# norlab-ulaval/norlab_icp_mapper

Measured on AMD Instinct MI355X. Metric: ICP iterations/sec, 100k-pt scan vs 1M-pt map, higher is better.
Workload: dtype f32; 1 GPU; single synthetic 100000-pt scan vs 1000000-pt map, point-to-point ICP, KDTreeMatcher knn 1 maxDist 2.0 epsilon 0, TrimmedDist 0.85, fixed 20 iterations per registration; chain=p2p, scene=box+pillars sigma=0.01 seeds 42/43/44 (SURVEY.md 8d), parallelism=scan-sharded x1, map replicated

## Files before the change

norlab_icp_mapper_amd/csrc/api.hip:

```cpp
#include "common.h"
#include <cstring>
#include <new>
#include <dlfcn.h>
#include <mutex>
#include <cstdio>

static std::string g_create_error;

namespace {
struct Roctx {
    int (*push)(const char*) = nullptr;
    int (*pop)() = nullptr;
    Roctx()
    {
        const char* e = getenv("ICPMI_ROCTX");
        if (!e || !atoi(e)) return;
        for (const char* name : {"librocprofiler-sdk-roctx.so.1", "librocprofiler-sdk-roctx.so", "/opt/rocm/lib/librocprofiler-sdk-roctx.so.1",
                                 "libroctx64.so.4", "libroctx64.so", "/opt/rocm/lib/libroctx64.so.4"}) {
            void* lib = dlopen(name, RTLD_NOW | RTLD_GLOBAL);
            if (!lib) continue;
            push = (int (*)(const char*))dlsym(lib, "roctxRangePushA");
            pop = (int (*)())dlsym(lib, "roctxRangePop");
            if (push && pop) return;
            push = nullptr; pop = nullptr;
// ... 213 lines not shown
icpmi_status icpmi_trim_cache(void)
{
    dev_cache_trim();
    return ICPMI_OK;
}


const char* icpmi_last_error(icpmi_handle h) { return h ? h->last_error.c_str() : g_create_error.c_str(); }

icpmi_status icpmi_set_stream(icpmi_handle h, void* hip_stream)
{
    CHECK_H(h);
    if (h->stream) hipStreamSynchronize(h->stream);
    if (h->own_stream && h->stream) stream_release(h->stream);
    h->stream = (hipStream_t)hip_stream;
    h->own_stream = false;
    drop_loop_graphs(h);
    return ICPMI_OK;
}

int32_t icpmi_has_map(icpmi_handle h) { return h && h->m > 0 ? 1 : 0; }

icpmi_status icpmi_get_map_mean(icpmi_handle h, float mean3[3])
{
    if (!h || !mean3) return ICPMI_ERR_INVALID_ARG;
    memcpy(mean3, h->mean, 3 * sizeof(float));
    return ICPMI_OK;
}

icpmi_status icpmi_debug_counters(icpmi_handle h, uint64_t out[24])
{
    if (!h || !out) return ICPMI_ERR_INVALID_ARG;
    for (int i = 0; i < 24; ++i) out[i] = h->h_state->dbg[i];
#ifndef ICPMI_NN_TIMING
    out[14] = (uint64_t)h->merge_fast_epochs;
    out[15] = (uint64_t)h->merge_slow_epochs;
    out[16] = (uint64_t)h->oct_respeculated;
    out[17] = (uint64_t)h->raw_view_count;
    out[18] = (uint64_t)(uint32_t)h->ins_count | ((uint64_t)(uint32_t)(h->temp_raw ? h->temp_raw->ins_count : 0) << 32);
    out[19] = (uint64_t)(uint32_t)h->full_count | ((uint64_t)(uint32_t)(h->temp_raw ? h->temp_raw->full_count : 0) << 32);
    out[20] = (uint64_t)h->normals_incremental;
    out[21] = (uint64_t)h->normals_full;
    out[22] = (uint64_t)h->normals_last_searched;
#endif
    return ICPMI_OK;
}

icpmi_status icpmi_debug_last_matches(icpmi_handle h, int64_t n, int32_t k, int32_t* ids, float* d2, float T_used[16])
{
    CHECK_H(h);
    if (n < 1 || k < 1 || !ids || !d2 || !T_used) { h->last_error = "debug_last_matches: bad arguments"; return ICPMI_ERR_INVALID_ARG; }
    if (h->last_match_n == 0) {
        h->last_error = "debug_last_matches: no single registration's matches on this handle (none ran, it failed, or a batch / another call came after it)";
        return ICPMI_ERR_UNSUPPORTED;
    }
    if (n != h->last_match_n || k != h->last_match_k) { h->last_error = "debug_last_matches: n / k differ from the last registration's"; return ICPMI_ERR_INVALID_ARG; }
    const size_t cnt = (size_t)n * k;
    DevBuf<int> d_ids;
    HIP_TRY(h, d_ids.alloc(cnt));
    icpmi_status s = nn_ids_to_original(h, h->d_sidx, (int64_t)cnt, d_ids);
    if (s != ICPMI_OK) return s;
    std::vector<int> hid(cnt), hq(h->last_match_sorted ? (size_t)n : 0);
    std::vector<float> hd(cnt);
    HIP_TRY(h, hipMemcpyAsync(hid.data(), d_ids, cnt * sizeof(int), hipMemcpyDeviceToHost, h->stream));
    HIP_TRY(h, hipMemcpyAsync(hd.data(), h->d_d2, cnt * sizeof(float), hipMemcpyDeviceToHost, h->stream));
    if (h->last_match_sorted) HIP_TRY(h, hipMemcpyAsync(hq.data(), h->d_qindex, (size_t)n * sizeof(int), hipMemcpyDeviceToHost, h->stream));
    HIP_TRY(h, hipMemcpyAsync(T_used, h->d_state->T_prev, 16 * sizeof(float), hipMemcpyDeviceToHost, h->stream));
// ... 766 lines not shown
```

norlab_icp_mapper_amd/csrc/common.h:

```cpp
#pragma once

#include <hip/hip_runtime.h>
#include <stdint.h>
#include <math.h>
#include <cstring>
#include <string>
#include <vector>
#include <unordered_map>
#include <mutex>
#include <map>
#include <cstdlib>
#include <shared_mutex>

#include "../../include/icpmi.h"

#define ICPMI_NV 32
#define ICPMI_MAX_OUTLIER 8
#define ICPMI_MAX_SMOOTH 16
#define ICPMI_SEL_BINS 2048
#ifndef ICPMI_S2_COPIES
#define ICPMI_S2_COPIES 8
#endif
#define ICPMI_S2_C0 4096
#define ICPMI_S2_F0 (ICPMI_S2_C0 + ICPMI_S2_COPIES * 256)
// ... 121 lines not shown
    int   stop_reason;
    int   counter;
    int   hist_n;
    double hq[(ICPMI_MAX_SMOOTH + 1) * 4];
    double ht[(ICPMI_MAX_SMOOTH + 1) * 3];
    double hrot[ICPMI_MAX_SMOOTH + 1];
    double htr[ICPMI_MAX_SMOOTH + 1];
    double init_q[4];
    unsigned sel_prefix;
    unsigned sel_rank;
    unsigned n_valid;
    unsigned sel_prefix_l[3];
    unsigned sel_rank_l[3];
    float limits[ICPMI_MAX_OUTLIER];
    unsigned vt_valid;
    float vt_ratio;
    float robust_med;
    float robust_scale;
    long long pairs;
    double wsum;
    unsigned hard_count;
    unsigned ticket;
    unsigned long long hard_total;
    unsigned seq;
    unsigned long long dbg[24];
    float T_prev[16];
    float T_out[16];
    unsigned long long t_start, t_done;
    unsigned long long t_nn_begin, t_nn_sum;
    unsigned nn_count, pad_nn;
};

#ifdef __HIPCC__
__device__ __forceinline__ void nn_stamp_open(IcpState* st) { st->t_nn_begin = (unsigned long long)wall_clock64(); }
__device__ __forceinline__ void nn_stamp_close(IcpState* st)
{
    const unsigned long long b = st->t_nn_begin;
    if (b) { st->t_nn_sum += (unsigned long long)wall_clock64() - b; ++st->nn_count; st->t_nn_begin = 0; }
}
#endif


inline std::shared_mutex& capture_gate() { static std::shared_mutex* m = new std::shared_mutex; return *m; }
struct CaptureGate {
    CaptureGate() { capture_gate().lock_shared(); }
    ~CaptureGate() { capture_gate().unlock_shared(); }
    CaptureGate(const CaptureGate&) = delete;
    CaptureGate& operator=(const CaptureGate&) = delete;
};

struct LoopGraph {
    hipGraphExec_t exec = nullptr; uint64_t sig = 0; int uses = 0; bool sorted = false;
    int len = 0; unsigned long used = 0;
    bool holds(uint64_t s) const { return exec && sig == s; }
    void reset() { if (exec) hipGraphExecDestroy(exec); *this = LoopGraph(); }
};
struct LoopGraphs {
    LoopGraph fixed, batch, seg[2], heads[4];
    unsigned long clock = 0;
    void reset() { fixed.reset(); batch.reset(); for (LoopGraph& g : seg) g.reset(); for (LoopGraph& g : heads) g.reset(); }
};

struct DevBlockCache {
    struct Live { size_t bytes; int dev; };
    std::mutex mu;
    std::unordered_map<void*, Live> live;
    std::map<int, std::multimap<size_t, void*>> idle_of;
// ... 616 lines not shown
```

norlab_icp_mapper_amd/csrc/loop.hip:

```cpp
#include "common.h"
#include "solve.h"
#include <cstring>

namespace {

template <int PASS, int MODE = 0>
__global__ __launch_bounds__(256) void sel_hist_kernel(const float* __restrict__ d2, int64_t count,
                                                       const IcpState* __restrict__ st, unsigned* __restrict__ ghist, int nb_scale = 0)
{
    if (st->done) return;
    if (blockIdx.x == 0 && threadIdx.x == 0) nn_stamp_close(const_cast<IcpState*>(st));
    if (MODE != 0 && nb_scale != 0 && st->iter + 1 > nb_scale) return;
    if (MODE == 3 && st->iter != 0) return;
    __shared__ unsigned h[ICPMI_SEL_BINS];
    for (int b = threadIdx.x; b < ICPMI_SEL_BINS; b += 256) h[b] = 0;
    __syncthreads();
    const unsigned prefix = st->sel_prefix;
    const float med = MODE == 2 ? st->robust_med : 0.f;
    for (int64_t i = (int64_t)blockIdx.x * 256 + threadIdx.x; i < count; i += (int64_t)gridDim.x * 256) {
        float v = d2[i];
        if (MODE == 0 || MODE == 3) { if (!(v != INFINITY && v > 0.f)) continue; }
        else {
            if (v == INFINITY) continue;
            if (MODE == 2) v = fabsf(v - med);
// ... 268 lines not shown
    for (int u = 0; u < PF; ++u) add(pv[u]);
    for (int64_t i = i0 + PF * stride; i < count; i += stride) add(d2[i]);
    __syncthreads();
    for (int i = threadIdx.x; i < WIN; i += 256) {
        const unsigned cnt = win[i];
        if (cnt) { const unsigned bin = lo + (unsigned)i; atomicAdd(&h[bin >> 8], cnt); atomicAdd(&fine[ICPMI_S2_FIDX(bin)], cnt); }
    }
    __syncthreads();
    if (h[threadIdx.x]) atomicAdd(&hists[ICPMI_S2_C0 + (blockIdx.x % ICPMI_S2_COPIES) * 256 + threadIdx.x], h[threadIdx.x]);
}

__global__ __launch_bounds__(256) void sel2_scan_hist_kernel(const float* __restrict__ d2, BatchArgs ba, int k, IcpState* __restrict__ st,
                                                             unsigned* __restrict__ hists, float quantile, int use_win)
{
    const int64_t count = (int64_t)ba.n[blockIdx.y] * k;
    d2 += (size_t)blockIdx.y * (size_t)ba.qstride * k;
    hists += (size_t)blockIdx.y * ICPMI_SELHIST_WORDS;
    st += blockIdx.y;
    constexpr int PF = 2;
    const int64_t stride = (int64_t)gridDim.x * 256;
    const int64_t i0 = (int64_t)blockIdx.x * 256 + threadIdx.x;
    float pv[PF];
#pragma unroll
    for (int u = 0; u < PF; ++u) pv[u] = i0 + u * stride < count ? d2[i0 + u * stride] : INFINITY;
    unsigned cv = 0;
#pragma unroll
    for (int cpy = 0; cpy < ICPMI_S2_COPIES; ++cpy) cv += hists[ICPMI_S2_C0 + cpy * 256 + threadIdx.x];
    if (st->done) return;
    if (blockIdx.x == 0 && threadIdx.x == 0) nn_stamp_close(const_cast<IcpState*>(st));
    __shared__ unsigned sh[16];
    unsigned prefix, rem, total;
    const bool win_hit = use_win && win_lookup(hists, quantile, sh, prefix, rem, total);
    if (!win_hit) block_find_rank_2tier<ICPMI_S2_FCOPIES>(cv, hists + ICPMI_S2_F0, true, quantile, 0u, sh, prefix, rem, total);
#ifndef ICPMI_NN_TIMING
    if (use_win && blockIdx.x == 0 && threadIdx.x == 0) st->dbg[win_hit ? 12 : 13] += 1ull;
#endif
    if (total == 0) {
        if (blockIdx.x == 0 && threadIdx.x == 0) { st->n_valid = 0; st->error = ICPMI_ERR_NO_OUTLIER_TO_FILTER; st->done = 1; }
        return;
    }
    if (blockIdx.x == 0 && threadIdx.x == 0) { st->sel_prefix_l[0] = prefix; st->sel_rank_l[0] = rem; st->n_valid = total; }
    auto add = [&](float v) {
        if (!(v != INFINITY && v > 0.f)) return;
        const unsigned bits = __float_as_uint(v);
        if ((bits >> 16) != prefix) return;
        atomicAdd(&hists[ICPMI_S2_C1 + ((bits >> 8) & 255u)], 1u);
        atomicAdd(&hists[ICPMI_S2_F1 + ICPMI_S2_FIDX(bits & 0xffffu)], 1u);
    };
#pragma unroll
    for (int u = 0; u < PF; ++u) add(pv[u]);
    for (int64_t i = i0 + PF * stride; i < count; i += stride) add(d2[i]);
}

constexpr int VT_CHUNK = 2048;

__global__ __launch_bounds__(256) void vt_keys_kernel(const float* __restrict__ d2, int64_t count, IcpState* __restrict__ st,
                                                      unsigned long long* __restrict__ keys, unsigned* __restrict__ vals)
{
    const int64_t i = (int64_t)blockIdx.x * 256 + threadIdx.x;
    if (blockIdx.x == 0 && threadIdx.x == 0 && !st->done) nn_stamp_close(st);
    const float v = i < count ? d2[i] : INFINITY;
    const bool valid = v != INFINITY && v > 0.f;
    if (i < count) { keys[i] = valid ? (unsigned long long)__float_as_uint(v) : 0xffffffffull; vals[i] = 0u; }
    __shared__ unsigned cnt;
    if (threadIdx.x == 0) cnt = 0;
    __syncthreads();
    const unsigned long long b = __ballot(valid);
// ... 1537 lines not shown
```

norlab_icp_mapper_amd/csrc/nn.hip:

```cpp
#include "common.h"

namespace {

constexpr int NN_BLOCK = 256;

typedef __attribute__((address_space(1))) unsigned gunsigned;
__device__ __forceinline__ float sqrt_up(float x) { return __builtin_amdgcn_sqrtf(x) * 1.0000005f; }
typedef float vf4 __attribute__((ext_vector_type(4)));
typedef __attribute__((address_space(1))) vf4 gfloat4;

struct Cand {
    unsigned long long key;
    int sidx;
};

__device__ __forceinline__ void cand_min(Cand& a, unsigned long long key, int sidx)
{
    if (key < a.key) { a.key = key; a.sidx = sidx; }
}

template <int G>
__device__ __forceinline__ void group_reduce(Cand& c)
{
#pragma unroll
// ... 249 lines not shown
__global__ __launch_bounds__(256) void ids_kernel(const float4* __restrict__ map, const int* __restrict__ sidx, int64_t count,
                                                  int* __restrict__ ids)
{
    const int64_t i = (int64_t)blockIdx.x * 256 + threadIdx.x;
    if (i >= count) return;
    const int s = sidx[i];
    ids[i] = s < 0 ? -1 : (int)__float_as_uint(map[s].w);
}

#ifdef ICPMI_NN_TIMING
#define NN_TICK(i) do { __builtin_amdgcn_s_waitcnt(0); const long long t_ = clock64(); tacc[i] += t_ - tlast; tlast = t_; } while (0)
#else
#define NN_TICK(i) do { } while (0)
#endif
__device__ __forceinline__ unsigned wave_incl_scan(unsigned v)
{
    v += (unsigned)__builtin_amdgcn_update_dpp(0, (int)v, 0x111, 0xf, 0xf, false);
    v += (unsigned)__builtin_amdgcn_update_dpp(0, (int)v, 0x112, 0xf, 0xf, false);
    v += (unsigned)__builtin_amdgcn_update_dpp(0, (int)v, 0x114, 0xf, 0xf, false);
    v += (unsigned)__builtin_amdgcn_update_dpp(0, (int)v, 0x118, 0xf, 0xf, false);
    v += (unsigned)__builtin_amdgcn_update_dpp(0, (int)v, 0x142, 0xa, 0xf, false);
    v += (unsigned)__builtin_amdgcn_update_dpp(0, (int)v, 0x143, 0xc, 0xf, false);
    return v;
}

#ifndef ICPMI_NN1_WAVES
#define ICPMI_NN1_WAVES 7
#endif
#if ICPMI_NN1_WAVES > 0
#define NN1_WAVES_ATTR __attribute__((amdgpu_waves_per_eu(ICPMI_NN1_WAVES, ICPMI_NN1_WAVES)))
#else
#define NN1_WAVES_ATTR
#endif
template <int NW, bool SELF>
__global__ __launch_bounds__(64 * NW) NN1_WAVES_ATTR void nn1_wg_kernel(const float4* __restrict__ queries, const int* __restrict__ qindex, BatchArgs ba,
                                                     const float* __restrict__ Tptr, GridLevels L, float maxr2, int* __restrict__ out_sidx,
                                                     float* __restrict__ out_d2, IcpState* __restrict__ st, unsigned* __restrict__ hard,
                                                     unsigned* __restrict__ hist0, float4* __restrict__ match_pt,
                                                     const uint4* __restrict__ ltab_g, int unseeded_lev, int seed_pre, float inv1e, float err2)
{
    static_assert(NW == 3 || NW == 4, "waves per workgroup");
    constexpr int NT = 64 * NW, Q = 64;
    constexpr int NR = 3;
    constexpr int CAP = 16 * Q;
#ifndef ICPMI_NN1_PLB
#define ICPMI_NN1_PLB 4
#endif
    constexpr int PLB = ICPMI_NN1_PLB;
    const int n = ba.n[blockIdx.y];
    {
        const size_t qo = (size_t)blockIdx.y * (size_t)ba.qstride;
        queries += qo; out_sidx += qo; out_d2 += qo;
        if (qindex) qindex += qo;
        if (match_pt) match_pt += qo;
        if (hist0) hist0 += (size_t)blockIdx.y * ICPMI_SELHIST_WORDS;
        if (Tptr) Tptr = reinterpret_cast<const float*>(reinterpret_cast<const char*>(Tptr) + (size_t)blockIdx.y * sizeof(IcpState));
        st += blockIdx.y;
    }
#ifdef ICPMI_NN_TIMING
    long long tacc[8] = {0, 0, 0, 0, 0, 0, 0, 0};
    long long tlast = clock64();
    const long long t_c0 = tlast, t_w0 = wall_clock64();
#endif
    __shared__ uint4 ltab[ICPMI_MAXLEV * 4];
    __shared__ unsigned lh[256];
    __shared__ uint2 pieces[CAP];
    __shared__ float2 qdec[Q];
    __shared__ float4 qrec[Q];
    __shared__ float2 qaux[Q];
    __shared__ unsigned long long qkey[Q];
    __shared__ unsigned qwin[Q];
    __shared__ float4 qpt[Q];
    __shared__ unsigned s_any, s_total[2];
    const int tid = threadIdx.x;
    const int lane = tid & 63;
    const int wave = tid >> 6;
    const bool w0 = wave == 0;
#ifndef ICPMI_NN_NO_HOIST
    {
        const GridParams g0 = L.g[0];
        asm volatile("" ::"s"(queries), "s"(qindex), "s"(out_sidx), "s"(out_d2), "s"(match_pt), "s"(ltab_g), "s"(Tptr), "s"(st), "s"(hist0), "s"(hard));
        asm volatile("" ::"s"(g0.ox), "s"(g0.oy), "s"(g0.oz), "s"(g0.cell), "s"(g0.inv_cell), "s"(g0.slack), "s"(L.nlev), "s"(maxr2), "s"(unseeded_lev), "s"(seed_pre), "s"(inv1e), "s"(err2));
    }
#endif
    const int wgs = (int)((((long long)n + Q - 1) / Q + 7) / 8 * 8);
    if ((int)blockIdx.x >= wgs) return;
    const int chunk = wgs >> 3;
    const int lb = (blockIdx.x & 7) * chunk + (blockIdx.x >> 3);
    const int slot = lane;
    const int qi = lb * Q + slot;
    const bool active = w0 && qi < n;
    float4 r = make_float4(0.f, 0.f, 0.f, 1.f);
    int orig = 0, sp_kept = -1;
    float4 qs_kept = make_float4(0.f, 0.f, 0.f, 0.f);
    if (w0) {
        r = ld_stream(queries + (active ? qi : 0));
        orig = match_pt ? qi : (qindex ? qindex[active ? qi : 0] : qi);
        if (match_pt) { sp_kept = ld_stream(out_sidx + (active ? qi : 0)); qs_kept = ld_stream(match_pt + (active ? qi : 0)); }
    }
    const int st_done = st->done, st_iter = st->iter;
    uint4 ltab_mine = make_uint4(0u, 0u, 0u, 0u);
    if (tid < ICPMI_MAXLEV * 4) ltab_mine = ltab_g[tid];
    float3 p = make_float3(0.f, 0.f, 0.f);
    if (w0) {
        if (Tptr) p = xf_point(Tptr, r.x, r.y, r.z, r.w);
        else p = make_float3(r.x, r.y, r.z);
    }
    if (st_done) return;
    if (blockIdx.x == 0 && threadIdx.x == 0) nn_stamp_open(st);
    if (tid < ICPMI_MAXLEV * 4) ltab[tid] = ltab_mine;
    if (hist0) {
        for (int t = tid; t < 256; t += NT) lh[t] = 0;
        for (int gt = blockIdx.x * NT + tid; gt < 256 + 65536; gt += wgs * NT) hist0[ICPMI_S2_C1 + gt] = 0;
    }
    const bool allow_self = SELF;

    Cand best; best.key = ~0ull; best.sidx = -1;
    bool decided = !active;
    int lev0 = unseeded_lev;
    if (w0) {
        int sp = -1;
        float4 qs = make_float4(0.f, 0.f, 0.f, 0.f);
        if (active && allow_self && st_iter > 0) {
            sp = match_pt ? sp_kept : out_sidx[orig];
            if (sp >= 0) qs = match_pt ? qs_kept : L.pts[0][sp];
        }
        bool want = sp >= 0;
        const float ub2 = sqdist3(p.x, p.y, p.z, qs.x, qs.y, qs.z);
        const float ub = sqrt_up(ub2);
        auto try_level = [&](int lev, const GridParams& gl) {
            const float fx = (p.x - gl.ox) * gl.inv_cell, fy = (p.y - gl.oy) * gl.inv_cell, fz = (p.z - gl.oz) * gl.inv_cell;
            float mfl = fminf(fx - floorf(fx), 1.0f - (fx - floorf(fx)));
            mfl = fminf(mfl, fminf(fy - floorf(fy), 1.0f - (fy - floorf(fy))));
            mfl = fminf(mfl, fminf(fz - floorf(fz), 1.0f - (fz - floorf(fz))));
            if (!(mfl >= 0.f)) mfl = 0.f;
            const float margin = (1.0f + mfl) * gl.cell - 2.0f * gl.slack;
            if (want && ub * inv1e * 1.000001f <= margin) {
                lev0 = lev;
                best.key = pack_key(ub2, __float_as_uint(qs.w));
                best.sidx = sp;
                qpt[slot] = qs;
                want = false;
            }
        };
        try_level(0, L.g[0]);
        for (int lev = 1; lev < L.nlev; ++lev) {
            if (__ballot(want) == 0ull) break;
            try_level(lev, L.g[lev]);
        }
    }
    bool widepre = false;
    if (seed_pre && lev0 > 0 && best.key != ~0ull) { widepre = true; lev0 = 0; }

    int lev = lev0;
    bool did_pre = false;
    if (w0) { qrec[slot] = make_float4(p.x, p.y, p.z, __int_as_float(lev0)); qkey[slot] = best.key; qwin[slot] = (unsigned)best.sidx; }
    NN_TICK(0);
    __syncthreads();
    for (;;) {
        bool run = false, prescan = false;
        if (w0) {
            run = !decided && lev < L.nlev;
            const bool any = __ballot(run) != 0ull;
            if (lane == 0) { s_any = any ? 1u : 0u; s_total[0] = 0u; s_total[1] = 0u; }
            if (any) {
                const int lv = run ? lev : 0;
                const unsigned long long bk = qkey[slot];
                prescan = run && !did_pre && (bk == ~0ull || (widepre && lev == 0));
                float rub2 = INFINITY;
                if (!prescan && bk != ~0ull) {
                    const float slack = __uint_as_float(ltab[4 * lv + 1].y);
                    const float rub = sqrt_up(__uint_as_float((unsigned)(bk >> 32))) * inv1e * 1.000001f + slack;
                    rub2 = rub * rub;
                }
                reinterpret_cast<float*>(&qrec[slot])[3] = __int_as_float(lv);
                qaux[slot] = make_float2(rub2, __int_as_float((run ? 1 : 0) | (prescan ? 2 : 0)));
            }
        }
        __syncthreads();
        if (!s_any) break;
        NN_TICK(1);
        {
            float mf, g_cell, g_slack;
            bool covers;
            const float4 qr = qrec[slot];
            const float2 qa = qaux[slot];
            const int lv = __float_as_int(qr.w);
            const int fl = __float_as_int(qa.y);
            const bool qrun = (fl & 1) != 0, qpre = (fl & 2) != 0;
            const float rub2 = qa.x;
            GridParams g;
            const gunsigned* __restrict__ cs;
            {
                const uint4 a = ltab[4 * lv], b = ltab[4 * lv + 1], c2 = ltab[4 * lv + 2], d = ltab[4 * lv + 3];
                g.ox = __uint_as_float(a.x); g.oy = __uint_as_float(a.y); g.oz = __uint_as_float(a.z); g.cell = __uint_as_float(a.w);
                g.inv_cell = __uint_as_float(b.x); g.slack = __uint_as_float(b.y); g.nx = (int)b.z; g.ny = (int)b.w;
                g.nz = (int)c2.x; g.ncells = (int)c2.y;
                cs = reinterpret_cast<const gunsigned*>(((unsigned long long)d.y << 32) | d.x);
            }
            const float fx = (qr.x - g.ox) * g.inv_cell, fy = (qr.y - g.oy) * g.inv_cell, fz = (qr.z - g.oz) * g.inv_cell;
            const float flx = floorf(fx), fly = floorf(fy), flz = floorf(fz);
            const int cx = (int)fminf(fmaxf(flx, -1.0e6f), 1.0e6f);
            const int cy = (int)fminf(fmaxf(fly, -1.0e6f), 1.0e6f);
            const int cz = (int)fminf(fmaxf(flz, -1.0e6f), 1.0e6f);
            mf = fminf(fx - flx, 1.0f - (fx - flx));
            mf = fminf(mf, fminf(fy - fly, 1.0f - (fy - fly)));
            mf = fminf(mf, fminf(fz - flz, 1.0f - (fz - flz)));
            if (!(mf >= 0.f)) mf = 0.f;
            g_cell = g.cell; g_slack = g.slack;
            covers = cx - 1 <= 0 && cx + 1 >= g.nx - 1 && cy - 1 <= 0 && cy + 1 >= g.ny - 1 && cz - 1 <= 0 && cz + 1 >= g.nz - 1;
            if (w0) { const float margin = fmaxf((1.0f + mf) * g_cell - g_slack, 0.f); qdec[slot] = make_float2(margin * margin, covers ? 1.f : 0.f); }
            unsigned rs[NR], rn[NR];
            {
                const float ylo = (fy - fly) * g.cell, yhi = (1.0f - (fy - fly)) * g.cell;
                const float zlo = (fz - flz) * g.cell, zhi = (1.0f - (fz - flz)) * g.cell;
                unsigned ia[NR], ib[NR];
#pragma unroll
                for (int sl = 0; sl < NR; ++sl) {
                    const int rr = wave + sl * NW;
                    const int dy = (rr % 3) - 1, dz = (rr / 3) - 1;
                    bool reach = qrun && rr < 9 && (!qpre || rr == 4);
                    const float ddy = dy == 0 ? 0.f : (dy < 0 ? ylo : yhi);
                    const float ddz = dz == 0 ? 0.f : (dz < 0 ? zlo : zhi);
                    const float rem2 = rub2 - (ddy * ddy + ddz * ddz);
                    reach = reach && rem2 >= 0.f;
                    int xa = cx - 1, xb = cx + 1;
                    if (rem2 != INFINITY) {
                        const float rem = sqrt_up(fmaxf(rem2, 0.f));
                        const int xl = (int)fmaxf(floorf((qr.x - rem - g.ox) * g.inv_cell), -1.0e6f);
                        const int xh = (int)fminf(floorf((qr.x + rem - g.ox) * g.inv_cell), 1.0e6f);
                        xa = xl > xa ? xl : xa;
                        xb = xh < xb ? xh : xb;
                    }
                    const int y = cy + dy, z = cz + dz;
                    xa = xa < 0 ? 0 : xa;
                    xb = xb > g.nx - 1 ? g.nx - 1 : xb;
                    reach = reach && y >= 0 && y < g.ny && z >= 0 && z < g.nz && xa <= xb;
                    const int rowbase = (z * g.ny + y) * g.nx;
                    ia[sl] = reach ? (unsigned)(rowbase + xa) : 0u;
                    ib[sl] = reach ? (unsigned)(rowbase + xb + 1) : 0u;
                }
#pragma unroll
                for (int sl = 0; sl < NR; ++sl) { rs[sl] = cs[ia[sl]]; rn[sl] = cs[ib[sl]]; }
#pragma unroll
                for (int sl = 0; sl < NR; ++sl) rn[sl] -= rs[sl];
            }
            int plb = PLB;
            unsigned base = 0;
            for (int round = 0; round < 2; ++round) {
                unsigned np = 0;
#pragma unroll
                for (int sl = 0; sl < NR; ++sl) np += (rn[sl] + ((1u << plb) - 1u)) >> plb;
                const unsigned incl = wave_incl_scan(np);
                const unsigned wtot = (unsigned)__builtin_amdgcn_readlane((int)incl, 63);
                unsigned wb = 0;
                if (lane == 63 && wtot) wb = atomicAdd(&s_total[round], wtot);
                wb = (unsigned)__builtin_amdgcn_readlane((int)wb, 63);
                base = wb + incl - np;
                __syncthreads();
                const unsigned tot = s_total[round];
                if (tot <= (unsigned)CAP) break;
                int k = 1;
                while ((tot >> k) > (unsigned)(CAP - 9 * Q)) ++k;
                plb += k;
            }
#pragma unroll
            for (int sl = 0; sl < NR; ++sl) {
                unsigned s = rs[sl], c = rn[sl];
                while (c) {
                    const unsigned t = c < (1u << plb) ? c : (1u << plb);
                    pieces[base++] = make_uint2(s, (t << 8) | (unsigned)slot);
                    s += t; c -= t;
                }
            }
        }
        __syncthreads();
        const unsigned total = s_total[1] ? s_total[1] : s_total[0];
        NN_TICK(2);
#ifdef ICPMI_NN_TIMING
        tacc[6] += 1; tacc[7] += total;
#endif
        for (unsigned i0 = 0; i0 < total; i0 += (unsigned)NT) {
            const unsigned i = i0 + (unsigned)tid;
            const bool has = i < total;
            const uint2 e = pieces[has ? i : 0u];
            const unsigned qsl = e.y & 255u, cnt = has ? e.y >> 8 : 0u;
            const float4 qr = qrec[qsl];
            const uint4 lt2 = ltab[4 * __float_as_int(qr.w) + 2];
            const gfloat4* mp = reinterpret_cast<const gfloat4*>((((unsigned long long)lt2.w << 32) | lt2.z) + (unsigned long long)e.x * 16ull);
            unsigned long long kb = ~0ull;
            unsigned pb = 0;
            float bx = 0.f, by = 0.f, bz = 0.f;
            for (unsigned c0 = 0; c0 < cnt; c0 += 8u) {
                vf4 q[8];
#pragma unroll
                for (int u = 0; u < 8; ++u) q[u] = mp[c0 + u];
#pragma unroll
                for (int u = 0; u < 8; ++u) {
                    const float d2 = sqdist3(qr.x, qr.y, qr.z, q[u].x, q[u].y, q[u].z);
                    const unsigned long long key = pack_key(d2, __float_as_uint(q[u].w));
                    bool ok = c0 + (unsigned)u < cnt;
                    if (!allow_self) ok = ok && d2 > 1.1920929e-07f;
                    if (ok && key < kb) { kb = key; pb = c0 + (unsigned)u; bx = q[u].x; by = q[u].y; bz = q[u].z; }
                }
            }
            if (kb != ~0ull) atomicMin(&qkey[qsl], kb);
            __syncthreads();
            if (kb != ~0ull && __atomic_load_n(&qkey[qsl], __ATOMIC_RELAXED) == kb) {
                qwin[qsl] = (e.x + pb) | (__float_as_uint(qr.w) << 28);
                qpt[qsl] = make_float4(bx, by, bz, __uint_as_float((unsigned)(kb & 0xffffffffull)));
            }
        }
        __syncthreads();
        NN_TICK(3);
        if (w0 && run) {
            const unsigned long long k2 = qkey[slot];
            if (prescan) did_pre = true;
            else {
                const float2 dq = qdec[slot];
                const float m2 = dq.x;
                const bool covers = dq.y != 0.f;
                const float bd2 = __uint_as_float((unsigned)(k2 >> 32));
                decided = (k2 != ~0ull && bd2 <= m2 * err2) || m2 > maxr2 || covers;
                if (!decided) { ++lev; did_pre = false; }
            }
        }
        NN_TICK(4);
    }
    if (w0) { best.key = qkey[slot]; best.sidx = (int)qwin[slot]; }

    float bd2 = __uint_as_float((unsigned)(best.key >> 32));
    const bool found = best.key != ~0ull && bd2 <= maxr2;
    if (!found) bd2 = INFINITY;
    const bool writer = active;
    if (hist0) {
        if (writer && decided && bd2 != INFINITY && bd2 > 0.f) atomicAdd(&lh[__float_as_uint(bd2) >> 24], 1u);
        __syncthreads();
        for (int t = tid; t < 256; t += NT)
            if (lh[t]) atomicAdd(&hist0[ICPMI_S2_C0 + (blockIdx.x % ICPMI_S2_COPIES) * 256 + t], lh[t]);
    }
    if (writer) {
        int bs = -1;
        float4 mpt = make_float4(0.f, 0.f, 0.f, 0.f);
        if (found) {
            const unsigned lvb = (unsigned)best.sidx >> 28, pos = (unsigned)best.sidx & 0x0fffffffu;
            if (lvb == 0) bs = (int)pos;
            else {
                const uint4 d = ltab[4 * lvb + 3];
                bs = (int)reinterpret_cast<const unsigned*>(((unsigned long long)d.w << 32) | d.z)[pos];
            }
            mpt = qpt[slot];
        }
        st_stream(out_sidx + orig, bs);
        st_stream(out_d2 + orig, bd2);
        if (match_pt) st_stream(match_pt + orig, make_float4(mpt.x, mpt.y, mpt.z, __uint_as_float((unsigned)(best.key & 0xffffffffull))));
        if (hist0 && decided && bd2 != INFINITY && bd2 > 0.f) {
            const unsigned bits = __float_as_uint(bd2);
            atomicAdd(&hist0[ICPMI_S2_F0 + (blockIdx.x % ICPMI_S2_FCOPIES) * 65536 + ICPMI_S2_FIDX(bits >> 16)], 1u);
        }
        if (!decided) {
            const unsigned hslot = atomicAdd(&st->hard_count, 1u);
            hard[hslot] = (unsigned)(match_pt ? qi : (qindex ? qindex[qi] : qi));
        }
    }
#ifdef ICPMI_NN_TIMING
    NN_TICK(5);
    if (threadIdx.x == 0 && st_iter > 1 && (blockIdx.x % 7) == 0) {
        atomicMax(&st->dbg[20], (unsigned long long)(clock64() - t_c0));
        atomicMax(&st->dbg[21], (unsigned long long)tacc[7]);
    }
    if (threadIdx.x == 0 && (blockIdx.x % 61) == 0) {
        const int tb = st_iter > 1 ? 8 : 0;
        for (int i = 0; i < 6; ++i) atomicAdd(&st->dbg[tb + i], (unsigned long long)tacc[i]);
        atomicAdd(&st->dbg[tb + 6], (unsigned long long)tacc[6]);
        atomicAdd(&st->dbg[tb + 7], 1ull);
        atomicAdd(&st->dbg[16 + (st_iter > 1 ? 1 : 0)], (unsigned long long)tacc[7]);
        atomicAdd(&st->dbg[22], (unsigned long long)(clock64() - t_c0));
        atomicAdd(&st->dbg[23], (unsigned long long)(wall_clock64() - t_w0));
    }
#endif
}

template <int G, int KMAX>
__global__ __launch_bounds__(NN_BLOCK) void nnk_ml_kernel(const float4* __restrict__ queries, const int* __restrict__ qindex, int n,
                                                          const float* __restrict__ Tptr, const uint4* __restrict__ ltab_g, int nlev,
                                                          int k, float maxr2, int allow_self_i, int seeded, int* __restrict__ out_sidx,
                                                          float* __restrict__ out_d2, IcpState* __restrict__ st,
                                                          unsigned* __restrict__ hard, int out_sorted, float inv1e, float err2)
{
    static_assert(G == 8, "lanes per query");
    constexpr int NB = 4;
    constexpr int NR = (9 + G - 1) / G;
    if (st->done) return;
    if (blockIdx.x == 0 && threadIdx.x == 0) nn_stamp_open(st);
    __shared__ uint4 ltab[ICPMI_MAXLEV * 4];
    if (threadIdx.x < ICPMI_MAXLEV * 4) ltab[threadIdx.x] = ltab_g[threadIdx.x];
    const bool allow_self = allow_self_i != 0;
// ... 672 lines not shown
#endif
}

}

void nn_launch_hard_k1(icpmi_ctx* c, const float4* d_reading, const float* d_T, const LoopCfg& lc, int allow_self, int* d_sidx,
                       float* d_d2, IcpState* d_state)
{
    hipLaunchKernelGGL(nn1_hard_kernel, dim3(512), dim3(NN_BLOCK), 0, c->stream, d_reading, d_T, c->d_map_sorted, (int)c->m, lc.maxr2,
                       allow_self, d_sidx, d_d2, d_state, c->d_hard);
    hipLaunchKernelGGL(hard_reset_kernel, dim3(1), dim3(64), 0, c->stream, d_state);
}

icpmi_status nn_launch_k1(icpmi_ctx* c, const float4* d_reading, int64_t n, const float* d_T, const LoopCfg& lc, int allow_self,
                          int* d_sidx, float* d_d2, IcpState* d_state)
{
    c->nn_out_sorted = false;
    {
        const bool sorted = c->batch_cur > 1 || (c->qsorted_n == n && c->qsorted_src == d_reading);
        const float4* q = sorted ? c->d_qsorted : d_reading;
        const int* qi = sorted ? c->d_qindex : nullptr;
        if (n == 0) return ICPMI_OK;
        const GridParams& topg = c->levels.g[c->levels.nlev - 1];
        const bool needs_hard = !std::isfinite(lc.max_dist) || (topg.cell - topg.slack) <= lc.max_dist;
        const int unseeded_lev = 0;
        const bool hard_sorted = needs_hard && allow_self && sorted && c->batch_cur <= 1;
        unsigned* h0 = (needs_hard && !hard_sorted) ? nullptr : c->nn_hist0;
        c->nn_builds_hist0 = h0 != nullptr;
        float4* mp = ((needs_hard && !hard_sorted) || !sorted) ? nullptr : c->nn_match_pt;
        c->nn_out_sorted = mp != nullptr;
        const BatchArgs ba = c->batch_cur > 1 ? c->batch_args : batch_of_one(n);
        const bool seeded = c->nn_iter_hint > 0 && allow_self;
        const int seed_pre = (seeded && c->nn_iter_hint > 1) ? 0 : 1;
#define LAUNCH_WG(S_)                                                                                                           \
    hipLaunchKernelGGL((nn1_wg_kernel<4, S_>), dim3((int)(((n + 63) / 64 + 7) / 8 * 8), ba.nscan), dim3(256), 0, c->stream,    \
                       q, qi, ba, d_T, c->levels, lc.maxr2, d_sidx, d_d2, d_state, c->d_hard, h0, mp, c->d_lvl_tab, unseeded_lev, seed_pre, lc.inv1e, lc.err2)
        if (allow_self) LAUNCH_WG(true); else LAUNCH_WG(false);
#undef LAUNCH_WG
        const GridParams& top = c->levels.g[c->levels.nlev - 1];
        if (!std::isfinite(lc.max_dist) || (top.cell - top.slack) <= lc.max_dist) {
            if (hard_sorted && mp)
                hipLaunchKernelGGL(nn1_hard_kernel, dim3(512), dim3(NN_BLOCK), 0, c->stream, q, d_T, c->d_map_sorted, (int)c->m,
                                   lc.maxr2, allow_self, d_sidx, d_d2, d_state, c->d_hard, mp, c->nn_builds_hist0 ? c->nn_hist0 : (unsigned*)nullptr);
            else
            hipLaunchKernelGGL(nn1_hard_kernel, dim3(512), dim3(NN_BLOCK), 0, c->stream, d_reading, d_T, c->d_map_sorted, (int)c->m,
                               lc.maxr2, allow_self, d_sidx, d_d2, d_state, c->d_hard);
            if (!(hard_sorted && mp)) hipLaunchKernelGGL(hard_reset_kernel, dim3(1), dim3(64), 0, c->stream, d_state);
        }
        HIP_TRY(c, hipGetLastError());
        return ICPMI_OK;
    }
}

template <int KMAX>
static icpmi_status nnk_launch_t(icpmi_ctx* c, const float4* d_reading, int64_t n, const float* d_T, const LoopCfg& lc,
                                 int allow_self, int* d_sidx, float* d_d2, IcpState* d_state)
{
    if constexpr (KMAX <= 16) if (n > 0) {
        constexpr int KM = KMAX;
        {
            constexpr int G = 8;
            const bool sorted = c->qsorted_n == n && c->qsorted_src == d_reading;
            const float4* q = sorted ? c->d_qsorted : d_reading;
            const int* qi = sorted ? c->d_qindex : nullptr;
            const int seeded = (c->nn_iter_hint > 0 && allow_self) ? 3 : 0;
            const int grid = (int)(((n * G + NN_BLOCK - 1) / NN_BLOCK + 7) / 8 * 8);
            const GridParams& top = c->levels.g[c->levels.nlev - 1];
            const bool needs_hard = !std::isfinite(lc.max_dist) || (top.cell - top.slack) <= lc.max_dist;
            const int out_sorted = (c->nn_sorted_k && sorted && !needs_hard) ? 1 : 0;
            c->nn_out_sorted = out_sorted != 0;
// ... 61 lines not shown
```

norlab_icp_mapper_amd/csrc/solve.h:

```cpp
#pragma once
#include "common.h"

namespace {

__device__ void mat4_mul_dev(const float* A, const float* B, float* C)
{
    float R[16];
#pragma unroll
    for (int j = 0; j < 4; ++j)
#pragma unroll
        for (int i = 0; i < 4; ++i) {
            float s = A[i] * B[4 * j];
#pragma unroll
            for (int kk = 1; kk < 4; ++kk) s = fmaf(A[4 * kk + i], B[4 * j + kk], s);
            R[4 * j + i] = s;
        }
#pragma unroll
    for (int i = 0; i < 16; ++i) C[i] = R[i];
}

__device__ void jacobi_eig(int n, const double* Ain, double* w, double* Q)
{
    __shared__ double A[36];
    for (int i = 0; i < n * n; ++i) A[i] = Ain[i];
// ... 475 lines not shown
        const int RING = ICPMI_MAX_SMOOTH + 1;
        const int slot = st->hist_n % RING;
        quat_from_T(Ti, st->hq + 4 * slot);
        for (int r = 0; r < 3; ++r) st->ht[3 * slot + r] = Ti[12 + r];
        st->hist_n += 1;
        const int hn = st->hist_n;
        {
            const int a = (hn - 1) % RING, bq = (hn - 2) % RING;
            st->hrot[a] = fabs(quat_angdist(st->hq + 4 * a, st->hq + 4 * bq));
            const double dx = st->ht[3 * a] - st->ht[3 * bq], dy = st->ht[3 * a + 1] - st->ht[3 * bq + 1],
                         dz = st->ht[3 * a + 2] - st->ht[3 * bq + 2];
            st->htr[a] = sqrt(dx * dx + dy * dy + dz * dz);
        }
        if (hn > SL) {
            double rot = 0, tr = 0;
            for (int i = hn - 1; i >= hn - SL; --i) { rot += st->hrot[i % RING]; tr += st->htr[i % RING]; }
            rot /= SL; tr /= SL;
            if (rot != rot || tr != tr) { st->error = ICPMI_ERR_NAN; st->done = 1; return; }
            if (rot < (double)lc.min_rot && tr < (double)lc.min_trans) {
                if (iterate) reason = ICPMI_STOP_DIFFERENTIAL;
                iterate = false;
            }
        }
    }
    if (lc.use_bound) {
        __shared__ double q[4];
        quat_from_T(Ti, q);
        const double rot = fabs(quat_angdist(q, st->init_q));
        const double nt = sqrt((double)Ti[12] * Ti[12] + (double)Ti[13] * Ti[13] + (double)Ti[14] * Ti[14]);
        if (rot > (double)lc.max_rot || nt > (double)lc.max_trans) { st->error = ICPMI_ERR_BOUND; st->done = 1; return; }
    }
    if (!iterate) { st->done = 1; st->stop_reason = reason; }
    const long long tsolve3 = clock64();
#ifndef ICPMI_NN_TIMING
    st->dbg[20] += (unsigned long long)(tsolve3 - tsolve0);
    st->dbg[21] += 1;
    st->dbg[22] += (unsigned long long)(tsolve1 - tsolve0);
    st->dbg[23] += (unsigned long long)(tsolve3 - tsolve2);
#else
    (void)tsolve1; (void)tsolve2; (void)tsolve3;
#endif
}

__device__ void solve_body(IcpState* __restrict__ st, unsigned long long* __restrict__ acc, bool clear, const LoopCfg& lc,
                           float* __restrict__ T_step_out, double* __restrict__ sums_out)
{
    __shared__ double tot[ICPMI_NV];
    const int t = threadIdx.x;
    bool nonfinite = false;
    read_pair_sums(acc, tot, clear, &nonfinite, pair_sum_mask(lc));
    if (t < ICPMI_NV && sums_out) sums_out[t] = tot[t];
    if (nonfinite) { if (t == 0) { st->error = ICPMI_ERR_NAN; st->done = 1; } return; }
    if (t == 0) solve_serial(st, tot, lc, T_step_out);
}

__device__ __forceinline__ void publish_progress(const IcpState* st, unsigned* progress)
{
    if (!progress) return;
    const unsigned v = ((unsigned)(st->done != 0) << 31) | ((st->seq & 0x7ffffu) << 12) | ((unsigned)st->iter & 0xfffu);
    __hip_atomic_store(progress, v, __ATOMIC_RELEASE, __HIP_MEMORY_SCOPE_SYSTEM);
}
struct ProgressWord { bool mine, done; int iter; };
static inline ProgressWord decode_progress(unsigned v, unsigned seq) { return {((v >> 12) & 0x7ffffu) == seq, (v >> 31) != 0, (int)(v & 0xfffu)}; }


}
```

Measured before the change: 23850 iterations/s.

## Add FIRST-role NN1 kernel variant keeping per-query state in shared memory

Adds a FIRST template variant of the workgroup 1-NN kernel, used when self-match is disallowed or on unseeded/first-pass launches. It keeps per-query search state (level, prescan, decided) and the winner index in shared memory instead of registers, and precomputes a prescan row bound. After a prescan it skips re-scanning the centre row. The aim is to lower register pressure and avoid redundant centre-row work, at the cost of more shared-memory traffic and LDS usage. It also adds an optional NN timeline diagnostic behind a new macro.

Measured after the change: 23870 iterations/s, median of 4. No clear change (+0.1%).

```diff
diff --git a/norlab_icp_mapper_amd/csrc/api.hip b/norlab_icp_mapper_amd/csrc/api.hip
--- a/norlab_icp_mapper_amd/csrc/api.hip
+++ b/norlab_icp_mapper_amd/csrc/api.hip
@@ -269,7 +269,7 @@
 {
     if (!h || !out) return ICPMI_ERR_INVALID_ARG;
     for (int i = 0; i < 24; ++i) out[i] = h->h_state->dbg[i];
-#ifndef ICPMI_NN_TIMING
+#ifndef ICPMI_NN_DIAG
     out[14] = (uint64_t)h->merge_fast_epochs;
     out[15] = (uint64_t)h->merge_slow_epochs;
     out[16] = (uint64_t)h->oct_respeculated;
diff --git a/norlab_icp_mapper_amd/csrc/common.h b/norlab_icp_mapper_amd/csrc/common.h
--- a/norlab_icp_mapper_amd/csrc/common.h
+++ b/norlab_icp_mapper_amd/csrc/common.h
@@ -177,7 +177,17 @@
 };
 
 #ifdef __HIPCC__
-__device__ __forceinline__ void nn_stamp_open(IcpState* st) { st->t_nn_begin = (unsigned long long)wall_clock64(); }
+#if defined(ICPMI_NN_TIMING) || defined(ICPMI_NN_TIMELINE)
+#define ICPMI_NN_DIAG 1
+#endif
+__device__ __forceinline__ void nn_stamp_open(IcpState* st)
+{
+#ifdef ICPMI_NN_TIMELINE
+    __hip_atomic_store(&st->t_nn_begin, (unsigned long long)wall_clock64(), __ATOMIC_RELAXED, __HIP_MEMORY_SCOPE_AGENT);
+#else
+    st->t_nn_begin = (unsigned long long)wall_clock64();
+#endif
+}
 __device__ __forceinline__ void nn_stamp_close(IcpState* st)
 {
     const unsigned long long b = st->t_nn_begin;
diff --git a/norlab_icp_mapper_amd/csrc/loop.hip b/norlab_icp_mapper_amd/csrc/loop.hip
--- a/norlab_icp_mapper_amd/csrc/loop.hip
+++ b/norlab_icp_mapper_amd/csrc/loop.hip
@@ -324,7 +324,7 @@
     unsigned prefix, rem, total;
     const bool win_hit = use_win && win_lookup(hists, quantile, sh, prefix, rem, total);
     if (!win_hit) block_find_rank_2tier<ICPMI_S2_FCOPIES>(cv, hists + ICPMI_S2_F0, true, quantile, 0u, sh, prefix, rem, total);
-#ifndef ICPMI_NN_TIMING
+#ifndef ICPMI_NN_DIAG
     if (use_win && blockIdx.x == 0 && threadIdx.x == 0) st->dbg[win_hit ? 12 : 13] += 1ull;
 #endif
     if (total == 0) {
diff --git a/norlab_icp_mapper_amd/csrc/nn.hip b/norlab_icp_mapper_amd/csrc/nn.hip
--- a/norlab_icp_mapper_amd/csrc/nn.hip
+++ b/norlab_icp_mapper_amd/csrc/nn.hip
@@ -305,7 +305,7 @@
 #else
 #define NN1_WAVES_ATTR
 #endif
-template <int NW, bool SELF>
+template <int NW, bool SELF, bool FIRST>
 __global__ __launch_bounds__(64 * NW) NN1_WAVES_ATTR void nn1_wg_kernel(const float4* __restrict__ queries, const int* __restrict__ qindex, BatchArgs ba,
                                                      const float* __restrict__ Tptr, GridLevels L, float maxr2, int* __restrict__ out_sidx,
                                                      float* __restrict__ out_d2, IcpState* __restrict__ st, unsigned* __restrict__ hard,
@@ -335,10 +335,16 @@
     long long tlast = clock64();
     const long long t_c0 = tlast, t_w0 = wall_clock64();
 #endif
+#ifdef ICPMI_NN_TIMELINE
+    const unsigned long long tl_w0 = (unsigned long long)wall_clock64();
+    unsigned tl_pieces = 0;
+#endif
     __shared__ uint4 ltab[ICPMI_MAXLEV * 4];
     __shared__ unsigned lh[256];
     __shared__ uint2 pieces[CAP];
     __shared__ float2 qdec[Q];
+    __shared__ int qstate[FIRST ? Q : 1];
+    __shared__ float qrow[FIRST ? Q : 1];
     __shared__ float4 qrec[Q];
     __shared__ float2 qaux[Q];
     __shared__ unsigned long long qkey[Q];
@@ -389,6 +395,7 @@
     const bool allow_self = SELF;
 
     Cand best; best.key = ~0ull; best.sidx = -1;
+    if (FIRST && w0) qwin[slot] = ~0u;
     bool decided = !active;
     int lev0 = unseeded_lev;
     if (w0) {
@@ -411,7 +418,8 @@
             if (want && ub * inv1e * 1.000001f <= margin) {
                 lev0 = lev;
                 best.key = pack_key(ub2, __float_as_uint(qs.w));
-                best.sidx = sp;
+                if (FIRST) qwin[slot] = (unsigned)sp;
+                else best.sidx = sp;
                 qpt[slot] = qs;
                 want = false;
             }
@@ -427,12 +435,15 @@
 
     int lev = lev0;
     bool did_pre = false;
-    if (w0) { qrec[slot] = make_float4(p.x, p.y, p.z, __int_as_float(lev0)); qkey[slot] = best.key; qwin[slot] = (unsigned)best.sidx; }
+    constexpr int ST_PRE = 1 << 8, ST_WIDE = 1 << 9, ST_DEC = 1 << 10;
+    if (FIRST && w0) qstate[slot] = lev0 | (widepre ? ST_WIDE : 0) | (decided ? ST_DEC : 0);
+    if (w0) { qrec[slot] = make_float4(p.x, p.y, p.z, __int_as_float(lev0)); qkey[slot] = best.key; if (!FIRST) qwin[slot] = (unsigned)best.sidx; }
     NN_TICK(0);
     __syncthreads();
     for (;;) {
         bool run = false, prescan = false;
         if (w0) {
+            if (FIRST) { const int qst = qstate[slot]; lev = qst & 255; did_pre = (qst & ST_PRE) != 0; widepre = (qst & ST_WIDE) != 0; decided = (qst & ST_DEC) != 0; }
             run = !decided && lev < L.nlev;
             const bool any = __ballot(run) != 0ull;
             if (lane == 0) { s_any = any ? 1u : 0u; s_total[0] = 0u; s_total[1] = 0u; }
@@ -447,7 +458,19 @@
                     rub2 = rub * rub;
                 }
                 reinterpret_cast<float*>(&qrec[slot])[3] = __int_as_float(lv);
-                qaux[slot] = make_float2(rub2, __int_as_float((run ? 1 : 0) | (prescan ? 2 : 0)));
+                if (FIRST && prescan) {
+                    const uint4 a = ltab[4 * lv], b = ltab[4 * lv + 1];
+                    const float4 qr = qrec[slot];
+                    const float inv = __uint_as_float(b.x);
+                    const float fx = (qr.x - __uint_as_float(a.x)) * inv, fy = (qr.y - __uint_as_float(a.y)) * inv, fz = (qr.z - __uint_as_float(a.z)) * inv;
+                    float mfx = fminf(fx - floorf(fx), 1.0f - (fx - floorf(fx)));
+                    float myz = fminf(fminf(fy - floorf(fy), 1.0f - (fy - floorf(fy))), fminf(fz - floorf(fz), 1.0f - (fz - floorf(fz))));
+                    if (!(mfx >= 0.f)) mfx = 0.f;
+                    if (!(myz >= 0.f)) myz = 0.f;
+                    const float rowm = fmaxf(fminf(myz, 1.0f + mfx) * __uint_as_float(a.w) - __uint_as_float(b.y), 0.f);
+                    qrow[slot] = rowm * rowm;
+                }
+                qaux[slot] = make_float2(rub2, __int_as_float((run ? 1 : 0) | (prescan ? 2 : 0) | ((FIRST && run && did_pre) ? 4 : 0)));
             }
         }
         __syncthreads();
@@ -460,7 +483,7 @@
             const float2 qa = qaux[slot];
             const int lv = __float_as_int(qr.w);
             const int fl = __float_as_int(qa.y);
-            const bool qrun = (fl & 1) != 0, qpre = (fl & 2) != 0;
+            const bool qrun = (fl & 1) != 0, qpre = (fl & 2) != 0, qpost = FIRST && (fl & 4) != 0;
             const float rub2 = qa.x;
             GridParams g;
             const gunsigned* __restrict__ cs;
@@ -492,7 +515,7 @@
                 for (int sl = 0; sl < NR; ++sl) {
                     const int rr = wave + sl * NW;
                     const int dy = (rr % 3) - 1, dz = (rr / 3) - 1;
-                    bool reach = qrun && rr < 9 && (!qpre || rr == 4);
+                    bool reach = qrun && rr < 9 && (!qpre || rr == 4) && !(qpost && rr == 4);
                     const float ddy = dy == 0 ? 0.f : (dy < 0 ? ylo : yhi);
                     const float ddz = dz == 0 ? 0.f : (dz < 0 ? zlo : zhi);
                     const float rem2 = rub2 - (ddy * ddy + ddz * ddz);
@@ -553,6 +576,9 @@
 #ifdef ICPMI_NN_TIMING
         tacc[6] += 1; tacc[7] += total;
 #endif
+#ifdef ICPMI_NN_TIMELINE
+        tl_pieces += total;
+#endif
         for (unsigned i0 = 0; i0 < total; i0 += (unsigned)NT) {
             const unsigned i = i0 + (unsigned)tid;
             const bool has = i < total;
@@ -586,9 +612,23 @@
         }
         __syncthreads();
         NN_TICK(3);
+        if (FIRST) {
+            const int fl3 = w0 ? __float_as_int(qaux[slot].y) : 0;
+            run = (fl3 & 1) != 0; prescan = (fl3 & 2) != 0;
+        }
         if (w0 && run) {
             const unsigned long long k2 = qkey[slot];
-            if (prescan) did_pre = true;
+            if (FIRST) {
+                int qst = qstate[slot];
+                const float2 dq = qdec[slot];
+                const float m2 = prescan ? qrow[slot] : dq.x;
+                const float bd2 = __uint_as_float((unsigned)(k2 >> 32));
+                const bool dec = (k2 != ~0ull && bd2 <= m2 * err2) || (!prescan && (m2 > maxr2 || dq.y != 0.f));
+                if (dec) qst |= ST_DEC;
+                if (prescan) qst |= ST_PRE;
+                else if (!dec) qst = (qst & ~ST_PRE) + 1;
+                qstate[slot] = qst;
+            } else if (prescan) did_pre = true;
             else {
                 const float2 dq = qdec[slot];
                 const float m2 = dq.x;
@@ -600,7 +640,8 @@
         }
         NN_TICK(4);
     }
-    if (w0) { best.key = qkey[slot]; best.sidx = (int)qwin[slot]; }
+    if (w0) { best.key = qkey[slot]; if (!FIRST) best.sidx = (int)qwin[slot]; }
+    if (FIRST) decided = w0 ? (qstate[slot] & ST_DEC) != 0 : true;
 
     float bd2 = __uint_as_float((unsigned)(best.key >> 32));
     const bool found = best.key != ~0ull && bd2 <= maxr2;
@@ -616,6 +657,7 @@
         int bs = -1;
         float4 mpt = make_float4(0.f, 0.f, 0.f, 0.f);
         if (found) {
+            if (FIRST) best.sidx = (int)qwin[slot];
             const unsigned lvb = (unsigned)best.sidx >> 28, pos = (unsigned)best.sidx & 0x0fffffffu;
             if (lvb == 0) bs = (int)pos;
             else {
@@ -624,9 +666,11 @@
             }
             mpt = qpt[slot];
         }
-        st_stream(out_sidx + orig, bs);
-        st_stream(out_d2 + orig, bd2);
-        if (match_pt) st_stream(match_pt + orig, make_float4(mpt.x, mpt.y, mpt.z, __uint_as_float((unsigned)(best.key & 0xffffffffull))));
+        int orig_w = orig;
+        if (FIRST) asm volatile("" : "+v"(orig_w));
+        st_stream(out_sidx + orig_w, bs);
+        st_stream(out_d2 + orig_w, bd2);
+        if (match_pt) st_stream(match_pt + orig_w, make_float4(mpt.x, mpt.y, mpt.z, __uint_as_float((unsigned)(best.key & 0xffffffffull))));
         if (hist0 && decided && bd2 != INFINITY && bd2 > 0.f) {
             const unsigned bits = __float_as_uint(bd2);
             atomicAdd(&hist0[ICPMI_S2_F0 + (blockIdx.x % ICPMI_S2_FCOPIES) * 65536 + ICPMI_S2_FIDX(bits >> 16)], 1u);
@@ -636,6 +680,20 @@
             hard[hslot] = (unsigned)(match_pt ? qi : (qindex ? qindex[qi] : qi));
         }
     }
+#ifdef ICPMI_NN_TIMELINE
+    if (!FIRST && threadIdx.x == 0 && st_iter > 1 && (blockIdx.x % 7) == 0) {
+        const unsigned long long t_open = __hip_atomic_load(&st->t_nn_begin, __ATOMIC_RELAXED, __HIP_MEMORY_SCOPE_AGENT), tl_w1 = (unsigned long long)wall_clock64();
+        auto tl_bin = [&](int dist, unsigned long long v, unsigned width) {
+            const unsigned b = v / width < 11ull ? (unsigned)(v / width) : 11u;
+            const int ctr = dist * 12 + (int)b;
+            atomicAdd(&st->dbg[ctr >> 1], (ctr & 1) ? (1ull << 32) : 1ull);
+        };
+        tl_bin(0, tl_w0 > t_open ? tl_w0 - t_open : 0ull, 100u);
+        tl_bin(1, tl_w1 - tl_w0, 200u);
+        tl_bin(2, tl_w1 > t_open ? tl_w1 - t_open : 0ull, 200u);
+        tl_bin(3, (unsigned long long)tl_pieces, 64u);
+    }
+#endif
 #ifdef ICPMI_NN_TIMING
     NN_TICK(5);
     if (threadIdx.x == 0 && st_iter > 1 && (blockIdx.x % 7) == 0) {
@@ -1374,10 +1432,16 @@
         const BatchArgs ba = c->batch_cur > 1 ? c->batch_args : batch_of_one(n);
         const bool seeded = c->nn_iter_hint > 0 && allow_self;
         const int seed_pre = (seeded && c->nn_iter_hint > 1) ? 0 : 1;
-#define LAUNCH_WG(S_)                                                                                                           \
-    hipLaunchKernelGGL((nn1_wg_kernel<4, S_>), dim3((int)(((n + 63) / 64 + 7) / 8 * 8), ba.nscan), dim3(256), 0, c->stream,    \
+#ifndef ICPMI_NN1_ROLES
+#define ICPMI_NN1_ROLES 1
+#endif
+        const bool first_role = ICPMI_NN1_ROLES && seed_pre;
+#define LAUNCH_WG(S_, F_)                                                                                                       \
+    hipLaunchKernelGGL((nn1_wg_kernel<4, S_, F_>), dim3((int)(((n + 63) / 64 + 7) / 8 * 8), ba.nscan), dim3(256), 0, c->stream,    \
                        q, qi, ba, d_T, c->levels, lc.maxr2, d_sidx, d_d2, d_state, c->d_hard, h0, mp, c->d_lvl_tab, unseeded_lev, seed_pre, lc.inv1e, lc.err2)
-        if (allow_self) LAUNCH_WG(true); else LAUNCH_WG(false);
+        if (!allow_self) LAUNCH_WG(false, true);
+        else if (first_role) LAUNCH_WG(true, true);
+        else LAUNCH_WG(true, false);
 #undef LAUNCH_WG
         const GridParams& top = c->levels.g[c->levels.nlev - 1];
         if (!std::isfinite(lc.max_dist) || (top.cell - top.slack) <= lc.max_dist) {
diff --git a/norlab_icp_mapper_amd/csrc/solve.h b/norlab_icp_mapper_amd/csrc/solve.h
--- a/norlab_icp_mapper_amd/csrc/solve.h
+++ b/norlab_icp_mapper_amd/csrc/solve.h
@@ -531,7 +531,7 @@
     }
     if (!iterate) { st->done = 1; st->stop_reason = reason; }
     const long long tsolve3 = clock64();
-#ifndef ICPMI_NN_TIMING
+#ifndef ICPMI_NN_DIAG
     st->dbg[20] += (unsigned long long)(tsolve3 - tsolve0);
     st->dbg[21] += 1;
     st->dbg[22] += (unsigned long long)(tsolve1 - tsolve0);
```
